# junhong-3dv/s2m2

Measured on AMD Instinct MI355X. Metric: stereo pairs/sec, S-model 1216x1024 fp16 refine_iter=3 (ms/pair = 1000*n_gpus/value), higher is better.
Workload: dtype f16; 1 GPU; S-model 1216x1024 refine_iter=3 use_positivity=True, 1 pair(s) per GPU per step, random-init weights (seeded LeCun normal); pairs_per_gpu=1, parallelism=dp1 (pairs sharded, RCCL gather of outputs to rank 0)

## Files before the change

s2m2_amd/csrc/conv.hip:

```cpp
#include "common.h"
#include "conv_select.h"
#include "launch.h"
#include "plan.h"

#ifndef S2M2_CONV_DBG
#define S2M2_CONV_DBG 0
#endif
#include "epilogue.h"

#ifndef S2M2_ASYNC_LOADS
#define S2M2_ASYNC_LOADS 0
#endif

namespace s2m2 {

struct ConvArgs {
    const void* src[4];
    int src_c[4];
    int src_stride[4];
    int nsrc;
    const void* weight;
    const float* bias;
    void* out;
    int out_stride;
    int N, H, W, KH, KW, Cin, Cout;
    int stride, Ho, Wo;
    int act, epi;
    const void* aux0;
    const void* aux1;
    int aux0_stride, aux1_stride;
    float out_scale;
    int shuffle2;
    int korder;
    const void* zero;
    const float* ln_wsum;
    float ln_eps;
    int ksplit;
    const float* bias2;
    int pool2;
    int epi_cout0;
};

template <typename T, int BM_, int BN_, int WGM_, int PPR_ = 8, int NPF_ = 1, int NWAVES_ = 4>
struct ConvCfg {
    static constexpr int NT = 64 * NWAVES_;
    static constexpr int NPF = NPF_;
    static constexpr int BM = BM_, BN = BN_, WGM = WGM_, WGN = NWAVES_ / WGM_;
    static constexpr int VEC = 16 / sizeof(T);
    static constexpr int PPR = PPR_;
    static constexpr int RPI = NT / PPR;
    static constexpr int BK = PPR * VEC;
    static constexpr int RS = BK + VEC;
    static constexpr int KSTEPS = BK / 16;
    static constexpr int WM = BM / WGM, WN = BN / WGN;
    static constexpr int MT = WM / 32, NTL = WN / 32;
    static constexpr int A_IT = (BM + RPI - 1) / RPI, B_IT = (BN + RPI - 1) / RPI;
    static constexpr int CRS = BN + VEC;
    static constexpr size_t TILE_BYTES = (size_t)2 * (BM + BN) * RS * sizeof(T);
    static constexpr size_t STAGE_BYTES = (size_t)BM * CRS * sizeof(T);
    static constexpr size_t LDS_BYTES = TILE_BYTES > STAGE_BYTES ? TILE_BYTES : STAGE_BYTES;
    static_assert(WM % 32 == 0 && WN % 32 == 0, "wave tile must be whole 32x32 MFMA tiles");
// ... 59 lines not shown
            }
            aux_combine(v, epi, a0, a1);
        }
        long long opix = m;
        int oc = co;
        if (p.shuffle2) {
            const int sub = co / p.shuffle2;
            oc = co - sub * p.shuffle2;
            const int x = (int)(m % p.Wo);
            const long long t = m / p.Wo;
            const int y = (int)(t % p.Ho);
            const long long n = t / p.Ho;
            opix = (n * (2 * p.Ho) + 2 * y + (sub >> 1)) * (2LL * p.Wo) + 2 * x + (sub & 1);
        }
        if (!(S2M2_CONV_DBG & 32)) *reinterpret_cast<Vec16<T>*>(outp + opix * p.out_stride + oc) = v;
    }
}

struct LinearPix {
    long long m0, M;
    __device__ __forceinline__ bool operator()(int r, long long& m) const { m = m0 + r; return m < M; }
};
template <int PW = 32>
struct PatchPixT {
    int n, y0, x0, H, W;
    __device__ __forceinline__ bool operator()(int r, long long& m) const {
        const int py = r / PW;
        const int yy = y0 + py, xx = x0 + (r - py * PW);
        m = ((long long)n * H + yy) * W + xx;
        return yy < H && xx < W;
    }
};
using PatchPix = PatchPixT<32>;

template <typename CFG, typename T>
__device__ __forceinline__ void stage_tile_ln(const ConvArgs& p, const float16_t (&acc)[CFG::MT][CFG::NTL], T* Cs, const CoutRegs<CFG>& bias,
                                              int wm, int wn, int lane, const LnRow* ln, const CoutRegs<CFG>& wsum) {
    if (p.act == S2M2_ACT_GELU) stage_tile<CFG, T, S2M2_ACT_GELU, true>(acc, Cs, bias, p.out_scale, wm, wn, lane, ln, &wsum);
    else stage_tile<CFG, T, S2M2_ACT_NONE, true>(acc, Cs, bias, p.out_scale, wm, wn, lane, ln, &wsum);
}

template <typename CFG, typename T>
__device__ __forceinline__ void stage_tile_act(const ConvArgs& p, const float16_t (&acc)[CFG::MT][CFG::NTL], T* Cs, const CoutRegs<CFG>& bias,
                                               int wm, int wn, int lane) {
    switch (p.act) {
        case S2M2_ACT_GELU: stage_tile<CFG, T, S2M2_ACT_GELU>(acc, Cs, bias, p.out_scale, wm, wn, lane); break;
        case S2M2_ACT_RELU: stage_tile<CFG, T, S2M2_ACT_RELU>(acc, Cs, bias, p.out_scale, wm, wn, lane); break;
        case S2M2_ACT_SIGMOID: stage_tile<CFG, T, S2M2_ACT_SIGMOID>(acc, Cs, bias, p.out_scale, wm, wn, lane); break;
        case S2M2_ACT_TANH: stage_tile<CFG, T, S2M2_ACT_TANH>(acc, Cs, bias, p.out_scale, wm, wn, lane); break;
        default: stage_tile<CFG, T, S2M2_ACT_NONE>(acc, Cs, bias, p.out_scale, wm, wn, lane); break;
    }
}

template <int CH>
struct KCursor {
    int ky, kx, kc;
    __device__ __forceinline__ void init(const ConvArgs& p, int elem) {
        ky = 0; kx = 0;
        if (p.korder) { kc = elem % CH; step(p, elem / CH); }
        else { kc = elem; norm(p); }
    }
    __device__ __forceinline__ void norm(const ConvArgs& p) {
        while (kc >= p.Cin) { kc -= p.Cin; if (++kx == p.KW) { kx = 0; ++ky; } }
    }
    __device__ __forceinline__ void step(const ConvArgs& p, int n) {
        for (int i = 0; i < n; ++i) {
            if (++kx == p.KW) { kx = 0; kc += CH; if (kc >= p.Cin) { kc -= p.Cin; ++ky; } }
        }
    }
    template <int BK> __device__ __forceinline__ void advance(const ConvArgs& p) {
        if (p.korder) step(p, BK / CH);
        else { kc += BK; norm(p); }
    }
};

template <typename CFG, typename T, bool POOL = false>
struct ConvLoader {
    static constexpr bool V1A = (S2M2_ASYNC_LOADS & 2) != 0;
    static constexpr int NQ = POOL ? 4 : 1;
    static constexpr int VEC = CFG::VEC, BK = CFG::BK, RS = CFG::RS, BN = CFG::BN;
    int pc, lrow, Ktot;
    int apix[CFG::A_IT];
    unsigned tapmask[CFG::A_IT];
    const T* wrow[CFG::B_IT];
    KCursor<4 * VEC> cur;
    const T *s0, *s1, *s2, *s3;
    int st0, st1, st2, st3, c0n, c1n, c2n;
    raw16_t ra[CFG::NPF][CFG::A_IT * NQ], rb[CFG::NPF][CFG::B_IT];

    __device__ __forceinline__ void init(const ConvArgs& p, int tid, long long m0, int n0, long long M, int Ktot_) {
        pc = tid % CFG::PPR; lrow = tid / CFG::PPR; Ktot = Ktot_;
        s0 = static_cast<const T*>(p.src[0]); s1 = static_cast<const T*>(p.src[1]);
        s2 = static_cast<const T*>(p.src[2]); s3 = static_cast<const T*>(p.src[3]);
        st0 = p.src_stride[0]; st1 = p.src_stride[1]; st2 = p.src_stride[2]; st3 = p.src_stride[3];
        c0n = p.src_c[0]; c1n = c0n + p.src_c[1]; c2n = c1n + p.src_c[2];
        const int ph = p.KH / 2, pw = p.KW / 2;
#pragma unroll
        for (int it = 0; it < CFG::A_IT; ++it) {
            const long long m = m0 + lrow + CFG::RPI * it;
            apix[it] = 0; tapmask[it] = 0u;
            if (m < M && lrow + CFG::RPI * it < CFG::BM) {
                const unsigned mu = (unsigned)m;
                const unsigned t = mu / (unsigned)p.Wo;
                const int xo = (int)(mu - t * (unsigned)p.Wo);
                const unsigned n = t / (unsigned)p.Ho;
                const int y = (int)(t - n * (unsigned)p.Ho) * p.stride, x = xo * p.stride;
// ... 748 lines not shown

#ifndef S2M2_FRAG_TRACE
#define S2M2_FRAG_TRACE 0
#endif
#if S2M2_FRAG_TRACE
__device__ unsigned long long g_frag_trace[4096 * 4 * 10];
#define FRAG_T(slot)                                                                                                          \
    do {                                                                                                                      \
        if ((threadIdx.x & 63) == 0 && blockIdx.x < 4096 && blockIdx.y == 0) {                                                \
            unsigned long long* tr_ = g_frag_trace + ((size_t)blockIdx.x * 4 + (threadIdx.x >> 6)) * 10;                     \
            tr_[(slot)] = __builtin_amdgcn_s_memtime();                                                                       \
            if ((slot) == 0) {                                                                                                \
                tr_[7] = __builtin_amdgcn_s_memrealtime();                                                                    \
                tr_[9] = (unsigned long long)__builtin_amdgcn_s_getreg((4 << 0) | (0 << 6) | (31 << 11)) |                    \
                         ((unsigned long long)__builtin_amdgcn_s_getreg((20 << 0) | (0 << 6) | (3 << 11)) << 32);             \
            }                                                                                                                 \
            if ((slot) == 6) tr_[8] = __builtin_amdgcn_s_memrealtime();                                                       \
        }                                                                                                                     \
    } while (0)
#else
#define FRAG_T(slot)
#endif

template <typename T, int BN_, int CH_, int PH_ = 4, int PW_ = 32>
struct ConvCfgF {
    static_assert(sizeof(T) == 2, "the fragment-stream kernel is fp16 only");
    static constexpr int BM = PW_ * PH_, BN = BN_, PH = PH_, PW = PW_, WGM = 1, WGN = BN_ / 32;
    static constexpr int NWAVES = WGN, NT = 64 * NWAVES;
    static constexpr int VEC = 8, CH = CH_, KS = CH_ / 16;
    static constexpr int RS = CH + VEC;
    static constexpr int WM = BM, WN = 32, MT = BM / 32, NTL = 1;
    static_assert(BM % 32 == 0, "a patch is a whole number of 32-pixel MFMA tiles");
    static constexpr int MAXHALO = (PH + 2) * (PW + 2);
    static constexpr int PPX = CH / VEC;
    static constexpr int RPI = NT / PPX;
    static constexpr int A_IT = (MAXHALO + RPI - 1) / RPI;
    static constexpr int CRS = BN + VEC;
    static constexpr int AROWS = A_IT * RPI;
    static constexpr size_t A_BYTES = (size_t)AROWS * RS * sizeof(T);
    static constexpr size_t STAGE_BYTES = (size_t)BM * CRS * sizeof(T);
    static constexpr size_t LDS_BYTES = A_BYTES > STAGE_BYTES ? A_BYTES : STAGE_BYTES;
    static_assert(NT % PPX == 0 && KS >= 2 && KS % 2 == 0, "loader geometry");
};

template <typename CFG, typename T, int AUX>
__global__ __launch_bounds__(CFG::NT) void conv_frag_kernel(ConvArgs p, int tiles_x, int tiles_y) {
    constexpr int BN = CFG::BN, VEC = CFG::VEC, RS = CFG::RS, CH = CFG::CH, KS = CFG::KS, PH = CFG::PH, PW = CFG::PW;
    extern __shared__ __attribute__((aligned(16))) char smem[];
    T* Ah = reinterpret_cast<T*>(smem);
    T* Cs = reinterpret_cast<T*>(smem);

    const int tid = threadIdx.x, lane = tid & 63;
    const int wv = __builtin_amdgcn_readfirstlane(tid >> 6);
    const int hi = lane >> 5, l31 = lane & 31;
    int bx = blockIdx.x;
    const int tx = bx % tiles_x; bx /= tiles_x;
    const int ty = bx % tiles_y;
    const int n = bx / tiles_y;
    const int y0 = ty * PH, x0 = tx * PW;
    const int n0 = blockIdx.y * BN;
    const int HW_ = p.KW + PW - 1, HH_ = p.KH + PH - 1;
    const int nhalo = HW_ * HH_;
    const int ph = p.KH / 2, pw = p.KW / 2;
    const int ntap = p.KH * p.KW;
    const int nchunk = (p.Cin + CH - 1) / CH;
    const int nfrag = nchunk * ntap * KS;
    FRAG_T(0);
    const int pc = tid % CFG::PPX, prow = tid / CFG::PPX;
    int apix[CFG::A_IT];
#pragma unroll
    for (int it = 0; it < CFG::A_IT; ++it) {
        const int hp = prow + CFG::RPI * it;
        apix[it] = -1;
        if (hp < nhalo) {
            const int hy = hp / HW_, hx = hp - hy * HW_;
            const int yy = y0 - ph + hy, xx = x0 - pw + hx;
            if (yy >= 0 && yy < p.H && xx >= 0 && xx < p.W) apix[it] = (n * p.H + yy) * p.W + xx;
        }
    }
    const T* zp = static_cast<const T*>(p.zero);
    const T* const s0 = static_cast<const T*>(p.src[0]);
    const T* const s1 = static_cast<const T*>(p.src[1]);
    const T* const s2 = static_cast<const T*>(p.src[2]);
    const T* const s3 = static_cast<const T*>(p.src[3]);
    const int st0 = p.src_stride[0], st1 = p.src_stride[1], st2 = p.src_stride[2], st3 = p.src_stride[3];
    const int c0n = p.src_c[0], c1n = c0n + p.src_c[1], c2n = c1n + p.src_c[2];
    auto load_halo = [&](int chunk) __attribute__((always_inline)) {
        const int kc = chunk * CH + pc * VEC;
        const bool cvalid = kc < p.Cin;
        const T* sp = s0;
        unsigned ss = (unsigned)st0, c = (unsigned)kc;
        if (p.nsrc > 1) {
            const bool g0 = kc >= c0n, g1 = kc >= c1n, g2 = kc >= c2n;
            const long long d1 = (const char*)s1 - (const char*)s0, d2 = (const char*)s2 - (const char*)s1, d3 = (const char*)s3 - (const char*)s2;
            sp = reinterpret_cast<const T*>((const char*)s0 + ((g0 ? d1 : 0) + (g1 ? d2 : 0) + (g2 ? d3 : 0)));
            ss = (unsigned)(st0 + (g0 ? st1 - st0 : 0) + (g1 ? st2 - st1 : 0) + (g2 ? st3 - st2 : 0));
            c = (unsigned)(kc - ((g0 ? c0n : 0) + (g1 ? c1n - c0n : 0) + (g2 ? c2n - c1n : 0)));
        }
        raw16_t ra[CFG::A_IT];
#pragma unroll
        for (int it = 0; it < CFG::A_IT; ++it) {
            const unsigned e = __umul24((unsigned)apix[it], ss) + c;
            const T* src = (cvalid && apix[it] >= 0) ? sp + e : zp;
            ra[it] = global_load16(src);
        }
#pragma unroll
        for (int it = 0; it < CFG::A_IT; ++it)
            *reinterpret_cast<raw16_t*>(Ah + (size_t)(prow + CFG::RPI * it) * RS + pc * VEC) = ra[it];
    };

    const raw16_t* wf = static_cast<const raw16_t*>(p.weight) + ((size_t)(blockIdx.y * CFG::WGN + wv) * nfrag) * 64 + lane;
    raw16_t ring[KS];

    CoutRegs<CFG> bias;
    bias.load(p.bias, p.zero, p.Cout, n0, wv, lane);
    const PatchPixT<PW> pix{n, y0, x0, p.H, p.W};
    constexpr bool AUX_LATE = AUX != 0 && PW != 32;
    using AX = AuxRegs<CFG, T, AUX != 0 ? (AUX_LATE ? 10 : 8) : 4>;
    AX aux;
    const int epi_eff = (n0 < p.epi_cout0) ? (int)S2M2_EPI_NONE : p.epi;
    if constexpr (AUX != 0 && !AUX_LATE) aux.template prefetch<AUX == 1>(p, tid, n0, pix, epi_eff);
    float16_t acc[CFG::MT][CFG::NTL];
#pragma unroll
    for (int i = 0; i < CFG::MT; ++i)
#pragma unroll
        for (int r = 0; r < 16; ++r) acc[i][0][r] = 0.f;

#pragma unroll
    for (int s = 0; s < KS; ++s) global_load16_async(ring[s], wf + (size_t)(s < nfrag ? s : nfrag - 1) * 64);
    load_halo(0);
    __syncthreads();
    FRAG_T(1);
    int g = 0;
    int poff[CFG::MT];
#pragma unroll
    for (int i = 0; i < CFG::MT; ++i) {
        if constexpr (PW == 32) poff[i] = (i * HW_ + l31) * RS;
        else { const int q = 32 * i + l31, qy = q / PW; poff[i] = (qy * HW_ + (q - qy * PW)) * RS; }
    }
    auto tap_steps = [&](int ky, int kx) __attribute__((always_inline)) {
        const T* a = Ah + (size_t)(ky * HW_ + kx) * RS + hi * 8;
        Frag<T> xf[2][CFG::MT];
#pragma unroll
        for (int i = 0; i < CFG::MT; ++i) load_frag(xf[0][i], a + poff[i]);
#pragma unroll
        for (int kk = 0; kk < KS; ++kk) {
            if (kk + 1 < KS) {
#pragma unroll
                for (int i = 0; i < CFG::MT; ++i) load_frag(xf[(kk + 1) & 1][i], a + poff[i] + (kk + 1) * 16);
            }
            wait_vmcnt<KS - 2>();
            settle(ring[kk]);
            Frag<T> wfr;
            wfr.v = __builtin_bit_cast(half8_t, ring[kk]);
#pragma unroll
            for (int i = 0; i < CFG::MT; ++i) mma32(acc[i][0], wfr, xf[kk & 1][i]);
            {
                const int f = g + KS - 1;
                global_load16_async(ring[(kk + KS - 1) % KS], wf + (size_t)(f < nfrag ? f : nfrag - 1) * 64);
            }
            ++g;
        }
    };
    for (int chunk = 0; chunk < nchunk; ++chunk) {
        if (chunk > 0) {
            wait_vmcnt<0>();
            __syncthreads();
            load_halo(chunk);
            __syncthreads();
        }
        int ky = 0, kx = 0;
#pragma unroll 1
        for (int tap = 0; tap < ntap; ++tap) {
            tap_steps(ky, kx);
            if (++kx == p.KW) { kx = 0; ++ky; }
        }
    }
    wait_vmcnt<0>();
#pragma unroll
    for (int s = 0; s < KS; ++s) settle(ring[s]);

    if constexpr (AUX_LATE) aux.template prefetch<AUX == 1>(p, tid, n0, pix, epi_eff);
    FRAG_T(2);
    __syncthreads();
    FRAG_T(3);
    stage_tile_act<CFG, T>(p, acc, Cs, bias, 0, wv, lane);
    FRAG_T(4);
    __syncthreads();
    FRAG_T(5);
    store_tile<CFG, T>(p, Cs, tid, n0, aux, pix, epi_eff);
    FRAG_T(6);
}

template <typename T, int BN_>
struct ConvCfgP {
    static constexpr int BM = 64, BN = BN_, WGM = 2, WGN = 2, NT = 256;
    static constexpr int VEC = 16 / sizeof(T);
    static constexpr int BK = 8 * VEC;
    static constexpr int RS = BK + VEC;
    static constexpr int KSTEPS = BK / 16;
    static constexpr int WM = 32, WN = BN / 2, MT = 1, NTL = WN / 32;
    static constexpr int A_IT = 2;
    static constexpr int CRS = BN + VEC;
    static constexpr size_t A_BYTES = (size_t)2 * BM * RS * sizeof(T);
    static constexpr size_t C_BYTES = (size_t)BM * CRS * sizeof(T);
    static constexpr size_t w_bytes(int K) { return (size_t)BN * (K + VEC) * sizeof(T); }
    static constexpr size_t lds_bytes(int K) { return A_BYTES + C_BYTES + w_bytes(K); }
};

template <typename CFG, typename T>
__global__ __launch_bounds__(256) void conv_pw_kernel(ConvArgs p, int ntiles) {
    constexpr int BM = CFG::BM, BN = CFG::BN, VEC = CFG::VEC, RS = CFG::RS, BK = CFG::BK;
    extern __shared__ __attribute__((aligned(16))) char smem[];
    T* As = reinterpret_cast<T*>(smem);
    T* Cs = reinterpret_cast<T*>(smem + CFG::A_BYTES);
    T* Ws = reinterpret_cast<T*>(smem + CFG::A_BYTES + CFG::C_BYTES);
    const int K = p.Cin;
    const int WRS = K + VEC;
    const int nchunk = (K + BK - 1) / BK;

    const int tid = threadIdx.x, lane = tid & 63;
    const int wv = __builtin_amdgcn_readfirstlane(tid >> 6);
    const int wm = wv & 1, wn = wv >> 1;
    const int hi = lane >> 5, l31 = lane & 31;
    const long long M = (long long)p.N * p.H * p.W;
    const int n0 = blockIdx.y * BN;
    CoutRegs<CFG> bias;
    bias.load(p.bias, p.zero, p.Cout, n0, wn, lane);
    const T* zp = static_cast<const T*>(p.zero);
// ... 324 lines not shown
```

s2m2_amd/csrc/convblock.hip:

```cpp
#include "common.h"
#include "launch.h"
#include "plan.h"
#include "epilogue.h"
#include <stdlib.h>

namespace s2m2 {

struct CbArgs {
    const half_t* x; half_t* out;
    long long xs, os;
    int N, H, W, tiles_x, tiles_y;
    const raw16_t* w1; const raw16_t* w2;
    const raw16_t* wa; const raw16_t* wb;
    const float* b1; const float* b2; const float* ba; const float* bb;
    const void* zero;
};

template <int C_, int PH_>
struct CbCfg {
    static constexpr int C = C_, PH = PH_, PW = 32, NW = C_ / 32, NT = 64 * NW, KS = 8, CH = 128, NCHUNK = C_ / 128;
    static constexpr int IH = PH + 2, IW = PW + 2, NI = IH * IW, MT1 = (NI + 31) / 32;
    static constexpr int HH = PH + 4, HW = PW + 4, NHALO = HH * HW;
    static constexpr int RS = CH + 8, TRS = C + 8;
    static constexpr int PPX = CH / 8, RPI = NT / PPX, A_IT = (NHALO + RPI - 1) / RPI, AROWS = A_IT * RPI;
    static constexpr size_t A_BYTES = (size_t)AROWS * RS * 2;
    static constexpr size_t R_BYTES = (size_t)PH * 32 * TRS * 2;
    static constexpr size_t T_BYTES = (size_t)MT1 * 32 * TRS * 2;
    static constexpr size_t A_REGION = A_BYTES > R_BYTES ? A_BYTES : R_BYTES;
    static constexpr size_t OFF_T = (A_REGION + 15) / 16 * 16, OFF_B = OFF_T + T_BYTES, LDS_BYTES = OFF_B + 4 * C * 4;
    static_assert(LDS_BYTES <= 160 * 1024 && NT % PPX == 0, "conv block tile");
};

template <int MT, int KS>
__device__ __forceinline__ void cb_steps(float16_t (&acc)[MT], const half_t* a, const int (&poff)[MT], raw16_t (&ring)[KS], const raw16_t* wf,
                                         int& g, int nfrag) {
    Frag<half_t> xf[2][MT];
#pragma unroll
    for (int i = 0; i < MT; ++i) load_frag(xf[0][i], a + poff[i]);
#pragma unroll
    for (int kk = 0; kk < KS; ++kk) {
        if (kk + 1 < KS) {
#pragma unroll
            for (int i = 0; i < MT; ++i) load_frag(xf[(kk + 1) & 1][i], a + poff[i] + (kk + 1) * 16);
        }
        wait_vmcnt<KS - 2>();
        settle(ring[kk]);
        Frag<half_t> wfr;
        wfr.v = __builtin_bit_cast(half8_t, ring[kk]);
#pragma unroll
        for (int i = 0; i < MT; ++i) mma32(acc[i], wfr, xf[kk & 1][i]);
        {
            const int f = g + KS - 1;
            global_load16_async(ring[(kk + KS - 1) % KS], wf + (size_t)(f < nfrag ? f : nfrag - 1) * 64);
        }
        ++g;
    }
}

template <typename CFG>
__global__ __launch_bounds__(CFG::NT) void conv_block_kernel(CbArgs p) {
    constexpr int C = CFG::C, PH = CFG::PH, KS = CFG::KS, RS = CFG::RS, TRS = CFG::TRS, HW = CFG::HW, IW = CFG::IW, MT1 = CFG::MT1, NCHUNK = CFG::NCHUNK;
    extern __shared__ __attribute__((aligned(16))) char smem[];
    half_t* Ah = reinterpret_cast<half_t*>(smem);
    half_t* Rt = reinterpret_cast<half_t*>(smem);
    half_t* Tt = reinterpret_cast<half_t*>(smem + CFG::OFF_T);
    float* bvec = reinterpret_cast<float*>(smem + CFG::OFF_B);
    const int tid = threadIdx.x, lane = tid & 63, l31 = lane & 31, hi = lane >> 5;
    const int wv = __builtin_amdgcn_readfirstlane(tid >> 6);
    int bx = blockIdx.x;
    const int tx = bx % p.tiles_x; bx /= p.tiles_x;
    const int ty = bx % p.tiles_y;
    const int n = bx / p.tiles_y;
    const int y0 = ty * PH, x0 = tx * 32;

    for (int i = tid; i < 4 * C; i += CFG::NT) {
        const int k = i / C, c = i - k * C;
        const float* src = k == 0 ? p.b1 : k == 1 ? p.b2 : k == 2 ? p.ba : p.bb;
        bvec[i] = src ? src[c] : 0.f;
    }
    const int pc = tid % CFG::PPX, prow = tid / CFG::PPX;
    const half_t* zp = static_cast<const half_t*>(p.zero);
    auto load_halo = [&](int chunk) __attribute__((always_inline)) {
        raw16_t ra[CFG::A_IT];
#pragma unroll
        for (int it = 0; it < CFG::A_IT; ++it) {
            const int hp = prow + CFG::RPI * it;
            const int hy = hp / HW, hx = hp - hy * HW;
            const int yy = y0 - 2 + hy, xx = x0 - 2 + hx;
            const bool ok = hp < CFG::NHALO && yy >= 0 && yy < p.H && xx >= 0 && xx < p.W;
            const half_t* src = ok ? p.x + ((long long)(n * p.H + yy) * p.W + xx) * p.xs + chunk * CFG::CH + pc * 8 : zp;
            ra[it] = global_load16(src);
        }
#pragma unroll
        for (int it = 0; it < CFG::A_IT; ++it) *reinterpret_cast<raw16_t*>(Ah + (size_t)(prow + CFG::RPI * it) * RS + pc * 8) = ra[it];
    };

    const int nfrag1 = NCHUNK * 9 * KS;
    const raw16_t* wf1 = p.w1 + (size_t)wv * nfrag1 * 64 + lane;
    const raw16_t* wfa = p.wa + (size_t)wv * (C / 16) * 64 + lane;
    raw16_t ring[KS];
    float16_t acc1[MT1], accA[PH];
#pragma unroll
    for (int i = 0; i < MT1; ++i)
#pragma unroll
        for (int r = 0; r < 16; ++r) acc1[i][r] = 0.f;
#pragma unroll
    for (int i = 0; i < PH; ++i)
#pragma unroll
        for (int r = 0; r < 16; ++r) accA[i][r] = 0.f;
    int poff1[MT1], poffA[PH];
#pragma unroll
    for (int i = 0; i < MT1; ++i) {
        int q = 32 * i + l31;
        q = q < CFG::NI ? q : CFG::NI - 1;
        const int iy = q / IW, ix = q - iy * IW;
        poff1[i] = (iy * HW + ix) * RS + hi * 8;
    }
#pragma unroll
    for (int i = 0; i < PH; ++i) poffA[i] = ((i + 2) * HW + l31 + 2) * RS + hi * 8;
#pragma unroll
    for (int s = 0; s < KS - 1; ++s) global_load16_async(ring[s], wf1 + (size_t)s * 64);
    int g = 0;
#pragma unroll 1
    for (int chunk = 0; chunk < NCHUNK; ++chunk) {
        if (chunk > 0) {
            wait_vmcnt<0>();
            __syncthreads();
        }
        load_halo(chunk);
        __syncthreads();
        int ky = 0, kx = 0;
#pragma unroll 1
        for (int tap = 0; tap < 9; ++tap) {
            cb_steps<MT1, KS>(acc1, Ah + (ky * HW + kx) * RS, poff1, ring, wf1, g, nfrag1);
            if (++kx == 3) { kx = 0; ++ky; }
        }
        wait_vmcnt<0>();
        {
            raw16_t wr[KS];
#pragma unroll
            for (int s = 0; s < KS; ++s) wr[s] = global_load16(wfa + (size_t)(chunk * KS + s) * 64);
#pragma unroll
            for (int s = 0; s < KS; ++s) {
                Frag<half_t> wfr;
                wfr.v = __builtin_bit_cast(half8_t, wr[s]);
#pragma unroll
                for (int i = 0; i < PH; ++i) {
                    Frag<half_t> xf;
                    load_frag(xf, Ah + poffA[i] + s * 16);
                    mma32(accA[i], wfr, xf);
                }
            }
        }
    }
    wait_vmcnt<0>();
#pragma unroll
    for (int s = 0; s < KS; ++s) settle(ring[s]);
    const int nfrag2 = NCHUNK * 9 * KS;
    const raw16_t* wf2 = p.w2 + (size_t)wv * nfrag2 * 64 + lane;
    __syncthreads();
#pragma unroll
    for (int i = 0; i < MT1; ++i) {
        const int q = 32 * i + l31;
        const int iy = q / IW, ix = q - iy * IW;
        const int yy = y0 - 1 + iy, xx = x0 - 1 + ix;
        const bool inside = q < CFG::NI && yy >= 0 && yy < p.H && xx >= 0 && xx < p.W;
        half_t* trow = Tt + (size_t)q * TRS + wv * 32 + 4 * hi;
#pragma unroll
        for (int gq = 0; gq < 4; ++gq) {
            const float4_t bv = *reinterpret_cast<const float4_t*>(bvec + wv * 32 + 8 * gq + 4 * hi);
            float v[4];
#pragma unroll
            for (int e = 0; e < 4; ++e) v[e] = acc1[i][4 * gq + e] + bv[e];
            const float2_t r0 = fast_gelu16x2((float2_t){v[0], v[1]}), r1 = fast_gelu16x2((float2_t){v[2], v[3]});
            half4_t h = {from_f32<half_t>(r0.x * 1.0f), from_f32<half_t>(r0.y * 1.0f), from_f32<half_t>(r1.x * 1.0f), from_f32<half_t>(r1.y * 1.0f)};
            if (!inside) h = half4_t{(half_t)0.f, (half_t)0.f, (half_t)0.f, (half_t)0.f};
            *reinterpret_cast<half4_t*>(trow + 8 * gq) = h;
        }
    }
#pragma unroll
    for (int i = 0; i < PH; ++i) {
        half_t* rrow = Rt + (size_t)(32 * i + l31) * TRS + wv * 32 + 4 * hi;
#pragma unroll
        for (int gq = 0; gq < 4; ++gq) {
            const float4_t bv = *reinterpret_cast<const float4_t*>(bvec + 2 * C + wv * 32 + 8 * gq + 4 * hi);
            half4_t h;
#pragma unroll
            for (int e = 0; e < 4; ++e) h[e] = from_f32<half_t>(fmaxf(accA[i][4 * gq + e] + bv[e], 0.f) * 1.0f);
            *reinterpret_cast<half4_t*>(rrow + 8 * gq) = h;
        }
    }
#pragma unroll
    for (int s = 0; s < KS - 1; ++s) global_load16_async(ring[s], wf2 + (size_t)s * 64);
    __syncthreads();
    float16_t acc2[PH], accB[PH];
#pragma unroll
    for (int i = 0; i < PH; ++i)
#pragma unroll
        for (int r = 0; r < 16; ++r) { acc2[i][r] = 0.f; accB[i][r] = 0.f; }
    int poff2[PH];
#pragma unroll
    for (int i = 0; i < PH; ++i) poff2[i] = (i * IW + l31) * TRS + hi * 8;
    g = 0;
#pragma unroll 1
    for (int chunk = 0; chunk < NCHUNK; ++chunk) {
        int ky = 0, kx = 0;
#pragma unroll 1
        for (int tap = 0; tap < 9; ++tap) {
            cb_steps<PH, KS>(acc2, Tt + (ky * IW + kx) * TRS + chunk * CFG::CH, poff2, ring, wf2, g, nfrag2);
            if (++kx == 3) { kx = 0; ++ky; }
        }
    }
    wait_vmcnt<0>();
#pragma unroll
    for (int s = 0; s < KS; ++s) settle(ring[s]);
    {
        const raw16_t* wfb = p.wb + (size_t)wv * (C / 16) * 64 + lane;
#pragma unroll 1
        for (int c8 = 0; c8 < C / 16; c8 += KS) {
            raw16_t wr[KS];
#pragma unroll
            for (int s = 0; s < KS; ++s) wr[s] = global_load16(wfb + (size_t)(c8 + s) * 64);
#pragma unroll
            for (int s = 0; s < KS; ++s) {
                Frag<half_t> wfr;
                wfr.v = __builtin_bit_cast(half8_t, wr[s]);
#pragma unroll
                for (int i = 0; i < PH; ++i) {
                    Frag<half_t> xf;
                    load_frag(xf, Rt + (size_t)(32 * i + l31) * TRS + hi * 8 + (c8 + s) * 16);
                    mma32(accB[i], wfr, xf);
                }
            }
        }
    }
#pragma unroll
    for (int i = 0; i < PH; ++i) {
        const int yy = y0 + i, xx = x0 + l31;
        if (yy < p.H && xx < p.W) {
            half_t* orow = p.out + ((long long)(n * p.H + yy) * p.W + xx) * p.os + wv * 32 + 4 * hi;
#pragma unroll
            for (int gq = 0; gq < 4; ++gq) {
                const float4_t b2 = *reinterpret_cast<const float4_t*>(bvec + C + wv * 32 + 8 * gq + 4 * hi);
                const float4_t bb = *reinterpret_cast<const float4_t*>(bvec + 3 * C + wv * 32 + 8 * gq + 4 * hi);
                half4_t h;
#pragma unroll
                for (int e = 0; e < 4; ++e) {
                    const half_t m = from_f32<half_t>((acc2[i][4 * gq + e] + b2[e]) * 1.0f);
                    const half_t s1 = from_f32<half_t>((accB[i][4 * gq + e] + bb[e]) * 1.0f);
                    h[e] = from_f32<half_t>((float)m + (float)s1);
                }
                *reinterpret_cast<half4_t*>(orow + 8 * gq) = h;
            }
        }
    }
}

template <int C, int PH>
static int launch_cb(const CbArgs& a0, hipStream_t st) {
    using CFG = CbCfg<C, PH>;
    CbArgs a = a0;
    a.tiles_x = (a.W + 31) / 32;
    a.tiles_y = (a.H + PH - 1) / PH;
    return launch<conv_block_kernel<CFG>>("conv_block", dim3((unsigned)(a.N * a.tiles_x * a.tiles_y)), dim3(CFG::NT), CFG::LDS_BYTES, st, a);
}

}

extern "C" int s2m2_conv_block_supported(int C, int H, int W, int dtype) {
    return dtype == S2M2_F16 && (C == 128 || C == 256) && H >= 1 && W >= 1 && (long long)H * W <= 160 * 192;
}

static int conv_block_impl(const s2m2_convblock_desc* d, void* stream) {
    using namespace s2m2;
    S2M2_REQUIRE(d, "conv_block: null descriptor");
    S2M2_REQUIRE(d->dtype == S2M2_F16 && (d->C == 128 || d->C == 256), "conv_block: C=%d dtype=%d (fp16, C = 128 / 256)", d->C, d->dtype);
    S2M2_REQUIRE(d->x && d->out && d->x != d->out, "conv_block: x / out must be distinct non-null tensors");
    S2M2_REQUIRE(d->N > 0 && d->H > 0 && d->W > 0 && (long long)d->N * d->H * d->W < (1LL << 24), "conv_block: bad shape");
    S2M2_REQUIRE(d->x_stride >= d->C && d->x_stride % 8 == 0 && d->out_stride >= d->C && d->out_stride % 4 == 0, "conv_block: pixel strides");
    S2M2_REQUIRE(d->w_conv0 && d->w_conv2 && d->w_1x0 && d->w_1x2, "conv_block: null weight");
    CbArgs a;
    a.x = static_cast<const half_t*>(d->x); a.out = static_cast<half_t*>(d->out); a.xs = d->x_stride; a.os = d->out_stride;
    a.N = d->N; a.H = d->H; a.W = d->W;
    a.w1 = static_cast<const raw16_t*>(d->w_conv0); a.w2 = static_cast<const raw16_t*>(d->w_conv2);
    a.wa = static_cast<const raw16_t*>(d->w_1x0); a.wb = static_cast<const raw16_t*>(d->w_1x2);
    a.b1 = d->b_conv0; a.b2 = d->b_conv2; a.ba = d->b_1x0; a.bb = d->b_1x2;
    if (bind_zero_page(a, "conv_block")) return 1;
    hipStream_t st = static_cast<hipStream_t>(stream);
    if (d->C == 256) return launch_cb<256, 2>(a, st);
    const long long b4 = (long long)d->N * ((d->W + 31) / 32) * ((d->H + 3) / 4);
    return (d->patch_rows == 4 || (d->patch_rows != 2 && b4 >= 128)) ? launch_cb<128, 4>(a, st) : launch_cb<128, 2>(a, st);
}
extern "C" int s2m2_conv_block(const s2m2_convblock_desc* d, void* stream) {
    return s2m2::plan_dispatch_desc<s2m2_convblock_desc>("s2m2_conv_block", &conv_block_impl, d, stream);
}

S2M2_PLAN_DESC_ENTRY("s2m2_conv_block", conv_block_impl)
```

Measured before the change: 125.4 pairs/s.

## Switch fragment-streaming conv kernels to 16x16x32 MFMA with paired weight steps

```diff
diff --git a/s2m2_amd/csrc/conv.hip b/s2m2_amd/csrc/conv.hip
--- a/s2m2_amd/csrc/conv.hip
+++ b/s2m2_amd/csrc/conv.hip
@@ -7,6 +7,8 @@
 #define S2M2_CONV_DBG 0
 #endif
 #include "epilogue.h"
+#include "frag_stream.h"
+#include <type_traits>
 
 #ifndef S2M2_ASYNC_LOADS
 #define S2M2_ASYNC_LOADS 0
@@ -172,6 +174,17 @@
     }
 }
 
+template <typename CFG, typename T, int NTILE>
+__device__ __forceinline__ void stage_tile_act(const ConvArgs& p, const float4_t (&acc)[NTILE][2], T* Cs, const CoutRegs16& bias, int, int wn, int lane) {
+    switch (p.act) {
+        case S2M2_ACT_GELU: stage_tile16<CFG, T, S2M2_ACT_GELU>(acc, Cs, bias, p.out_scale, wn, lane); break;
+        case S2M2_ACT_RELU: stage_tile16<CFG, T, S2M2_ACT_RELU>(acc, Cs, bias, p.out_scale, wn, lane); break;
+        case S2M2_ACT_SIGMOID: stage_tile16<CFG, T, S2M2_ACT_SIGMOID>(acc, Cs, bias, p.out_scale, wn, lane); break;
+        case S2M2_ACT_TANH: stage_tile16<CFG, T, S2M2_ACT_TANH>(acc, Cs, bias, p.out_scale, wn, lane); break;
+        default: stage_tile16<CFG, T, S2M2_ACT_NONE>(acc, Cs, bias, p.out_scale, wn, lane); break;
+    }
+}
+
 template <int CH>
 struct KCursor {
     int ky, kx, kc;
@@ -1026,7 +1039,6 @@
 
     const int tid = threadIdx.x, lane = tid & 63;
     const int wv = __builtin_amdgcn_readfirstlane(tid >> 6);
-    const int hi = lane >> 5, l31 = lane & 31;
     int bx = blockIdx.x;
     const int tx = bx % tiles_x; bx /= tiles_x;
     const int ty = bx % tiles_y;
@@ -1086,7 +1098,9 @@
     const raw16_t* wf = static_cast<const raw16_t*>(p.weight) + ((size_t)(blockIdx.y * CFG::WGN + wv) * nfrag) * 64 + lane;
     raw16_t ring[KS];
 
-    CoutRegs<CFG> bias;
+    using FS = FragShape<FRAG_MFMA>;
+    constexpr int NTILE = CFG::BM / FS::PIX;
+    std::conditional_t<FRAG_MFMA == 16, CoutRegs16, CoutRegs<CFG>> bias;
     bias.load(p.bias, p.zero, p.Cout, n0, wv, lane);
     const PatchPixT<PW> pix{n, y0, x0, p.H, p.W};
     constexpr bool AUX_LATE = AUX != 0 && PW != 32;
@@ -1094,61 +1108,47 @@
     AX aux;
     const int epi_eff = (n0 < p.epi_cout0) ? (int)S2M2_EPI_NONE : p.epi;
     if constexpr (AUX != 0 && !AUX_LATE) aux.template prefetch<AUX == 1>(p, tid, n0, pix, epi_eff);
-    float16_t acc[CFG::MT][CFG::NTL];
-#pragma unroll
-    for (int i = 0; i < CFG::MT; ++i)
-#pragma unroll
-        for (int r = 0; r < 16; ++r) acc[i][0][r] = 0.f;
-
-#pragma unroll
-    for (int s = 0; s < KS; ++s) global_load16_async(ring[s], wf + (size_t)(s < nfrag ? s : nfrag - 1) * 64);
-    load_halo(0);
-    __syncthreads();
-    FRAG_T(1);
+    typename FS::acc_t acc[NTILE];
+#pragma unroll
+    for (int i = 0; i < NTILE; ++i) frag_zero<FRAG_MFMA>(acc[i]);
+
+    if constexpr (FRAG_MFMA == 32) {
+#pragma unroll
+        for (int s = 0; s < KS; ++s) global_load16_async(ring[s], wf + (size_t)(s < nfrag ? s : nfrag - 1) * 64);
+        load_halo(0);
+        __syncthreads();
+        FRAG_T(1);
+    }
     int g = 0;
-    int poff[CFG::MT];
-#pragma unroll
-    for (int i = 0; i < CFG::MT; ++i) {
-        if constexpr (PW == 32) poff[i] = (i * HW_ + l31) * RS;
-        else { const int q = 32 * i + l31, qy = q / PW; poff[i] = (qy * HW_ + (q - qy * PW)) * RS; }
-    }
-    auto tap_steps = [&](int ky, int kx) __attribute__((always_inline)) {
-        const T* a = Ah + (size_t)(ky * HW_ + kx) * RS + hi * 8;
-        Frag<T> xf[2][CFG::MT];
-#pragma unroll
-        for (int i = 0; i < CFG::MT; ++i) load_frag(xf[0][i], a + poff[i]);
-#pragma unroll
-        for (int kk = 0; kk < KS; ++kk) {
-            if (kk + 1 < KS) {
-#pragma unroll
-                for (int i = 0; i < CFG::MT; ++i) load_frag(xf[(kk + 1) & 1][i], a + poff[i] + (kk + 1) * 16);
-            }
-            wait_vmcnt<KS - 2>();
-            settle(ring[kk]);
-            Frag<T> wfr;
-            wfr.v = __builtin_bit_cast(half8_t, ring[kk]);
-#pragma unroll
-            for (int i = 0; i < CFG::MT; ++i) mma32(acc[i][0], wfr, xf[kk & 1][i]);
-            {
-                const int f = g + KS - 1;
-                global_load16_async(ring[(kk + KS - 1) % KS], wf + (size_t)(f < nfrag ? f : nfrag - 1) * 64);
-            }
-            ++g;
-        }
-    };
+    int poff[NTILE];
+    const int lpx = FS::pixel(lane), lko = FS::koff(lane);
+#pragma unroll
+    for (int i = 0; i < NTILE; ++i) {
+        const int q = FS::PIX * i + lpx, qy = q / PW;
+        poff[i] = (qy * HW_ + (q - qy * PW)) * RS + lko;
+    }
     for (int chunk = 0; chunk < nchunk; ++chunk) {
-        if (chunk > 0) {
-            wait_vmcnt<0>();
-            __syncthreads();
+        if constexpr (FRAG_MFMA == 32) {
+            if (chunk > 0) {
+                wait_vmcnt<0>();
+                __syncthreads();
+                load_halo(chunk);
+                __syncthreads();
+            }
+        } else {
+            if (chunk > 0) __syncthreads();
+            frag_prime<FRAG_MFMA, KS>(ring, wf, g, nfrag);
             load_halo(chunk);
             __syncthreads();
+            if (chunk == 0) FRAG_T(1);
         }
         int ky = 0, kx = 0;
 #pragma unroll 1
-        for (int tap = 0; tap < ntap; ++tap) {
-            tap_steps(ky, kx);
+        for (int tap = 0; tap < (FRAG_MFMA == 32 ? ntap : ntap - 1); ++tap) {
+            frag_steps<FRAG_MFMA, NTILE, KS>(acc, Ah + (size_t)(ky * HW_ + kx) * RS, poff, ring, wf, g, nfrag);
             if (++kx == p.KW) { kx = 0; ++ky; }
         }
+        if constexpr (FRAG_MFMA == 16) frag_steps<FRAG_MFMA, NTILE, KS, FRAG_MFMA == 16>(acc, Ah + (size_t)(ky * HW_ + kx) * RS, poff, ring, wf, g, nfrag);
     }
     wait_vmcnt<0>();
 #pragma unroll
diff --git a/s2m2_amd/csrc/convblock.hip b/s2m2_amd/csrc/convblock.hip
--- a/s2m2_amd/csrc/convblock.hip
+++ b/s2m2_amd/csrc/convblock.hip
@@ -2,6 +2,7 @@
 #include "launch.h"
 #include "plan.h"
 #include "epilogue.h"
+#include "frag_stream.h"
 #include <stdlib.h>
 
 namespace s2m2 {
@@ -26,46 +27,26 @@
     static constexpr size_t A_BYTES = (size_t)AROWS * RS * 2;
     static constexpr size_t R_BYTES = (size_t)PH * 32 * TRS * 2;
     static constexpr size_t T_BYTES = (size_t)MT1 * 32 * TRS * 2;
+    using FS = FragShape<FRAG_MFMA>;
+    static constexpr int NT1 = (NI + FS::PIX - 1) / FS::PIX;
+    static constexpr int NT2 = PH * 32 / FS::PIX;
+    static_assert(NT1 * FS::PIX <= MT1 * 32, "the intermediate's rows");
     static constexpr size_t A_REGION = A_BYTES > R_BYTES ? A_BYTES : R_BYTES;
     static constexpr size_t OFF_T = (A_REGION + 15) / 16 * 16, OFF_B = OFF_T + T_BYTES, LDS_BYTES = OFF_B + 4 * C * 4;
     static_assert(LDS_BYTES <= 160 * 1024 && NT % PPX == 0, "conv block tile");
 };
 
-template <int MT, int KS>
-__device__ __forceinline__ void cb_steps(float16_t (&acc)[MT], const half_t* a, const int (&poff)[MT], raw16_t (&ring)[KS], const raw16_t* wf,
-                                         int& g, int nfrag) {
-    Frag<half_t> xf[2][MT];
-#pragma unroll
-    for (int i = 0; i < MT; ++i) load_frag(xf[0][i], a + poff[i]);
-#pragma unroll
-    for (int kk = 0; kk < KS; ++kk) {
-        if (kk + 1 < KS) {
-#pragma unroll
-            for (int i = 0; i < MT; ++i) load_frag(xf[(kk + 1) & 1][i], a + poff[i] + (kk + 1) * 16);
-        }
-        wait_vmcnt<KS - 2>();
-        settle(ring[kk]);
-        Frag<half_t> wfr;
-        wfr.v = __builtin_bit_cast(half8_t, ring[kk]);
-#pragma unroll
-        for (int i = 0; i < MT; ++i) mma32(acc[i], wfr, xf[kk & 1][i]);
-        {
-            const int f = g + KS - 1;
-            global_load16_async(ring[(kk + KS - 1) % KS], wf + (size_t)(f < nfrag ? f : nfrag - 1) * 64);
-        }
-        ++g;
-    }
-}
-
 template <typename CFG>
 __global__ __launch_bounds__(CFG::NT) void conv_block_kernel(CbArgs p) {
-    constexpr int C = CFG::C, PH = CFG::PH, KS = CFG::KS, RS = CFG::RS, TRS = CFG::TRS, HW = CFG::HW, IW = CFG::IW, MT1 = CFG::MT1, NCHUNK = CFG::NCHUNK;
+    constexpr int C = CFG::C, PH = CFG::PH, KS = CFG::KS, RS = CFG::RS, TRS = CFG::TRS, HW = CFG::HW, IW = CFG::IW, NT1 = CFG::NT1, NT2 = CFG::NT2, NCHUNK = CFG::NCHUNK;
+    using FS = typename CFG::FS;
     extern __shared__ __attribute__((aligned(16))) char smem[];
     half_t* Ah = reinterpret_cast<half_t*>(smem);
     half_t* Rt = reinterpret_cast<half_t*>(smem);
     half_t* Tt = reinterpret_cast<half_t*>(smem + CFG::OFF_T);
     float* bvec = reinterpret_cast<float*>(smem + CFG::OFF_B);
     const int tid = threadIdx.x, lane = tid & 63, l31 = lane & 31, hi = lane >> 5;
+    const int lpx = FS::pixel(lane), lko = FS::koff(lane), lq = lane >> 4;
     const int wv = __builtin_amdgcn_readfirstlane(tid >> 6);
     int bx = blockIdx.x;
     const int tx = bx % p.tiles_x; bx /= p.tiles_x;
@@ -99,42 +80,42 @@
     const raw16_t* wf1 = p.w1 + (size_t)wv * nfrag1 * 64 + lane;
     const raw16_t* wfa = p.wa + (size_t)wv * (C / 16) * 64 + lane;
     raw16_t ring[KS];
-    float16_t acc1[MT1], accA[PH];
-#pragma unroll
-    for (int i = 0; i < MT1; ++i)
-#pragma unroll
-        for (int r = 0; r < 16; ++r) acc1[i][r] = 0.f;
+    typename FS::acc_t acc1[NT1];
+    float16_t accA[PH];
+#pragma unroll
+    for (int i = 0; i < NT1; ++i) frag_zero<FRAG_MFMA>(acc1[i]);
 #pragma unroll
     for (int i = 0; i < PH; ++i)
 #pragma unroll
         for (int r = 0; r < 16; ++r) accA[i][r] = 0.f;
-    int poff1[MT1], poffA[PH];
-#pragma unroll
-    for (int i = 0; i < MT1; ++i) {
-        int q = 32 * i + l31;
+    int poff1[NT1], poffA[PH];
+#pragma unroll
+    for (int i = 0; i < NT1; ++i) {
+        int q = FS::PIX * i + lpx;
         q = q < CFG::NI ? q : CFG::NI - 1;
         const int iy = q / IW, ix = q - iy * IW;
-        poff1[i] = (iy * HW + ix) * RS + hi * 8;
+        poff1[i] = (iy * HW + ix) * RS + lko;
     }
 #pragma unroll
     for (int i = 0; i < PH; ++i) poffA[i] = ((i + 2) * HW + l31 + 2) * RS + hi * 8;
-#pragma unroll
-    for (int s = 0; s < KS - 1; ++s) global_load16_async(ring[s], wf1 + (size_t)s * 64);
     int g = 0;
+    if constexpr (FRAG_MFMA == 32) frag_prime<FRAG_MFMA, KS>(ring, wf1, 0, nfrag1);
 #pragma unroll 1
     for (int chunk = 0; chunk < NCHUNK; ++chunk) {
         if (chunk > 0) {
             wait_vmcnt<0>();
             __syncthreads();
         }
+        if constexpr (FRAG_MFMA == 16) frag_prime<FRAG_MFMA, KS>(ring, wf1, g, nfrag1);
         load_halo(chunk);
         __syncthreads();
         int ky = 0, kx = 0;
 #pragma unroll 1
-        for (int tap = 0; tap < 9; ++tap) {
-            cb_steps<MT1, KS>(acc1, Ah + (ky * HW + kx) * RS, poff1, ring, wf1, g, nfrag1);
+        for (int tap = 0; tap < (FRAG_MFMA == 32 ? 9 : 8); ++tap) {
+            frag_steps<FRAG_MFMA, NT1, KS>(acc1, Ah + (ky * HW + kx) * RS, poff1, ring, wf1, g, nfrag1);
             if (++kx == 3) { kx = 0; ++ky; }
         }
+        if constexpr (FRAG_MFMA == 16) frag_steps<FRAG_MFMA, NT1, KS, FRAG_MFMA == 16>(acc1, Ah + (2 * HW + 2) * RS, poff1, ring, wf1, g, nfrag1);
         wait_vmcnt<0>();
         {
             raw16_t wr[KS];
@@ -160,22 +141,27 @@
     const raw16_t* wf2 = p.w2 + (size_t)wv * nfrag2 * 64 + lane;
     __syncthreads();
 #pragma unroll
-    for (int i = 0; i < MT1; ++i) {
-        const int q = 32 * i + l31;
+    for (int i = 0; i < NT1; ++i) {
+        const int q = FS::PIX * i + lpx;
         const int iy = q / IW, ix = q - iy * IW;
         const int yy = y0 - 1 + iy, xx = x0 - 1 + ix;
         const bool inside = q < CFG::NI && yy >= 0 && yy < p.H && xx >= 0 && xx < p.W;
-        half_t* trow = Tt + (size_t)q * TRS + wv * 32 + 4 * hi;
-#pragma unroll
-        for (int gq = 0; gq < 4; ++gq) {
-            const float4_t bv = *reinterpret_cast<const float4_t*>(bvec + wv * 32 + 8 * gq + 4 * hi);
+        constexpr int NQ = FRAG_MFMA == 32 ? 4 : 2, QS = 32 / NQ;
+        const int c0 = wv * 32 + 4 * (FRAG_MFMA == 32 ? hi : lq);
+        half_t* trow = Tt + (size_t)q * TRS + c0;
+#pragma unroll
+        for (int gq = 0; gq < NQ; ++gq) {
+            const float4_t bv = *reinterpret_cast<const float4_t*>(bvec + c0 + QS * gq);
             float v[4];
 #pragma unroll
-            for (int e = 0; e < 4; ++e) v[e] = acc1[i][4 * gq + e] + bv[e];
+            for (int e = 0; e < 4; ++e) {
+                if constexpr (FRAG_MFMA == 32) v[e] = acc1[i][0][4 * gq + e] + bv[e];
+                else v[e] = acc1[i][gq][e] + bv[e];
+            }
             const float2_t r0 = fast_gelu16x2((float2_t){v[0], v[1]}), r1 = fast_gelu16x2((float2_t){v[2], v[3]});
             half4_t h = {from_f32<half_t>(r0.x * 1.0f), from_f32<half_t>(r0.y * 1.0f), from_f32<half_t>(r1.x * 1.0f), from_f32<half_t>(r1.y * 1.0f)};
             if (!inside) h = half4_t{(half_t)0.f, (half_t)0.f, (half_t)0.f, (half_t)0.f};
-            *reinterpret_cast<half4_t*>(trow + 8 * gq) = h;
+            *reinterpret_cast<half4_t*>(trow + QS * gq) = h;
         }
     }
 #pragma unroll
@@ -191,25 +177,31 @@
         }
     }
 #pragma unroll
-    for (int s = 0; s < KS - 1; ++s) global_load16_async(ring[s], wf2 + (size_t)s * 64);
+    for (int s = 0; s < FS::primed(KS); ++s) global_load16_async(ring[s], wf2 + (size_t)s * 64);
     __syncthreads();
-    float16_t acc2[PH], accB[PH];
+    typename FS::acc_t acc2[NT2];
+    float16_t accB[PH];
+#pragma unroll
+    for (int i = 0; i < NT2; ++i) frag_zero<FRAG_MFMA>(acc2[i]);
 #pragma unroll
     for (int i = 0; i < PH; ++i)
 #pragma unroll
-        for (int r = 0; r < 16; ++r) { acc2[i][r] = 0.f; accB[i][r] = 0.f; }
-    int poff2[PH];
-#pragma unroll
-    for (int i = 0; i < PH; ++i) poff2[i] = (i * IW + l31) * TRS + hi * 8;
+        for (int r = 0; r < 16; ++r) accB[i][r] = 0.f;
+    int poff2[NT2];
+#pragma unroll
+    for (int i = 0; i < NT2; ++i) {
+        const int q = FS::PIX * i + lpx;
+        poff2[i] = ((q >> 5) * IW + (q & 31)) * TRS + lko;
+    }
     g = 0;
+    {
+        int ky = 0, kx = 0, coff = 0;
 #pragma unroll 1
-    for (int chunk = 0; chunk < NCHUNK; ++chunk) {
-        int ky = 0, kx = 0;
-#pragma unroll 1
-        for (int tap = 0; tap < 9; ++tap) {
-            cb_steps<PH, KS>(acc2, Tt + (ky * IW + kx) * TRS + chunk * CFG::CH, poff2, ring, wf2, g, nfrag2);
-            if (++kx == 3) { kx = 0; ++ky; }
-        }
+        for (int tap = 0; tap < NCHUNK * 9 - (FRAG_MFMA == 32 ? 0 : 1); ++tap) {
+            frag_steps<FRAG_MFMA, NT2, KS>(acc2, Tt + (ky * IW + kx) * TRS + coff, poff2, ring, wf2, g, nfrag2);
+            if (++kx == 3) { kx = 0; if (++ky == 3) { ky = 0; coff += CFG::CH; } }
+        }
+        if constexpr (FRAG_MFMA == 16) frag_steps<FRAG_MFMA, NT2, KS, FRAG_MFMA == 16>(acc2, Tt + (2 * IW + 2) * TRS + (NCHUNK - 1) * CFG::CH, poff2, ring, wf2, g, nfrag2);
     }
     wait_vmcnt<0>();
 #pragma unroll
@@ -234,6 +226,24 @@
             }
         }
     }
+    if constexpr (FRAG_MFMA == 16) {
+        __syncthreads();
+#pragma unroll
+        for (int i = 0; i < NT2; ++i) {
+            half_t* mrow = Tt + (size_t)(16 * i + lpx) * TRS + wv * 32 + 4 * lq;
+#pragma unroll
+            for (int gq = 0; gq < 2; ++gq) {
+                const float4_t b2 = *reinterpret_cast<const float4_t*>(bvec + C + wv * 32 + 16 * gq + 4 * lq);
+                half4_t h;
+#pragma unroll
+                for (int e = 0; e < 4; ++e) h[e] = from_f32<half_t>((acc2[i][gq][e] + b2[e]) * 1.0f);
+                *reinterpret_cast<half4_t*>(mrow + 16 * gq) = h;
+            }
+        }
+        __builtin_amdgcn_fence(__ATOMIC_RELEASE, "wavefront");
+        __builtin_amdgcn_wave_barrier();
+        __builtin_amdgcn_fence(__ATOMIC_ACQUIRE, "wavefront");
+    }
 #pragma unroll
     for (int i = 0; i < PH; ++i) {
         const int yy = y0 + i, xx = x0 + l31;
@@ -243,10 +253,13 @@
             for (int gq = 0; gq < 4; ++gq) {
                 const float4_t b2 = *reinterpret_cast<const float4_t*>(bvec + C + wv * 32 + 8 * gq + 4 * hi);
                 const float4_t bb = *reinterpret_cast<const float4_t*>(bvec + 3 * C + wv * 32 + 8 * gq + 4 * hi);
-                half4_t h;
+                half4_t h, m4;
+                if constexpr (FRAG_MFMA == 16) m4 = *reinterpret_cast<const half4_t*>(Tt + (size_t)(32 * i + l31) * TRS + wv * 32 + 4 * hi + 8 * gq);
 #pragma unroll
                 for (int e = 0; e < 4; ++e) {
-                    const half_t m = from_f32<half_t>((acc2[i][4 * gq + e] + b2[e]) * 1.0f);
+                    half_t m;
+                    if constexpr (FRAG_MFMA == 16) m = m4[e];
+                    else m = from_f32<half_t>((acc2[i][0][4 * gq + e] + b2[e]) * 1.0f);
                     const half_t s1 = from_f32<half_t>((accB[i][4 * gq + e] + bb[e]) * 1.0f);
                     h[e] = from_f32<half_t>((float)m + (float)s1);
                 }
diff --git a/s2m2_amd/csrc/frag_stream.h b/s2m2_amd/csrc/frag_stream.h
--- /dev/null
+++ b/s2m2_amd/csrc/frag_stream.h
@@ -0,0 +1,169 @@
+#pragma once
+#include "common.h"
+#include "epilogue.h"
+
+#ifndef S2M2_FRAG_MFMA
+#define S2M2_FRAG_MFMA 16
+#endif
+static_assert(S2M2_FRAG_MFMA == 16 || S2M2_FRAG_MFMA == 32, "S2M2_FRAG_MFMA: 16 (v_mfma_f32_16x16x32_f16) or 32 (v_mfma_f32_32x32x16_f16)");
+
+namespace s2m2 {
+
+constexpr int FRAG_MFMA = S2M2_FRAG_MFMA;
+
+template <int SHAPE> struct FragShape;
+template <> struct FragShape<32> {
+    static constexpr int PIX = 32;
+    typedef float16_t acc_t[1];
+    __device__ static __forceinline__ int pixel(int lane) { return lane & 31; }
+    __device__ static __forceinline__ int koff(int lane) { return (lane >> 5) * 8; }
+    static constexpr int primed(int ks) { return ks - 1; }
+};
+template <> struct FragShape<16> {
+    static constexpr int PIX = 16;
+    typedef float4_t acc_t[2];
+    __device__ static __forceinline__ int pixel(int lane) {
+        const int c = lane & 15;
+        return (c >= 4 && c < 12) ? 2 * (c - 4) : (c < 4 ? 2 * c + 1 : 2 * (c - 8) + 1);
+    }
+    __device__ static __forceinline__ int koff(int lane) { const int q = lane >> 4; return (q & 1) * 16 + (q >> 1) * 8; }
+    static constexpr int primed(int ks) { return ks - 2; }
+};
+
+template <int SHAPE> __device__ __forceinline__ void frag_zero(typename FragShape<SHAPE>::acc_t& a) {
+    if constexpr (SHAPE == 32) {
+#pragma unroll
+        for (int r = 0; r < 16; ++r) a[0][r] = 0.f;
+    } else {
+#pragma unroll
+        for (int r = 0; r < 4; ++r) { a[0][r] = 0.f; a[1][r] = 0.f; }
+    }
+}
+
+template <int SHAPE, int KS>
+__device__ __forceinline__ void frag_prime(raw16_t (&ring)[KS], const raw16_t* wf, int g, int nfrag) {
+#pragma unroll
+    for (int s = 0; s < FragShape<SHAPE>::primed(KS); ++s) global_load16_async(ring[s], wf + (size_t)(g + s < nfrag ? g + s : nfrag - 1) * 64);
+}
+
+__device__ __forceinline__ void frag_pair_swap(raw16_t& f0, raw16_t& f1) {
+#pragma unroll
+    for (int d = 0; d < 4; ++d) {
+        const float a0 = f0[d], a1 = f1[d];
+        const auto r = __builtin_amdgcn_permlane16_swap(__builtin_bit_cast(unsigned, a0), __builtin_bit_cast(unsigned, a1), false, false);
+        const unsigned u0 = r[0], u1 = r[1];
+        f0[d] = __builtin_bit_cast(float, u0);
+        f1[d] = __builtin_bit_cast(float, u1);
+    }
+}
+
+template <int SHAPE, int NTILE, int KS, bool LAST = false>
+__device__ __forceinline__ void frag_steps(typename FragShape<SHAPE>::acc_t (&acc)[NTILE], const half_t* a, const int (&poff)[NTILE], raw16_t (&ring)[KS],
+                                           const raw16_t* wf, int& g, int nfrag) {
+    if constexpr (SHAPE == 32) {
+        static_assert(!LAST, "the 32-wide loop keeps its ring in flight across taps and chunks");
+        Frag<half_t> xf[2][NTILE];
+#pragma unroll
+        for (int i = 0; i < NTILE; ++i) load_frag(xf[0][i], a + poff[i]);
+#pragma unroll
+        for (int kk = 0; kk < KS; ++kk) {
+            if (kk + 1 < KS) {
+#pragma unroll
+                for (int i = 0; i < NTILE; ++i) load_frag(xf[(kk + 1) & 1][i], a + poff[i] + (kk + 1) * 16);
+            }
+            wait_vmcnt<KS - 2>();
+            settle(ring[kk]);
+            Frag<half_t> wfr;
+            wfr.v = __builtin_bit_cast(half8_t, ring[kk]);
+#pragma unroll
+            for (int i = 0; i < NTILE; ++i) mma32(acc[i][0], wfr, xf[kk & 1][i]);
+            {
+                const int f = g + KS - 1;
+                global_load16_async(ring[(kk + KS - 1) % KS], wf + (size_t)(f < nfrag ? f : nfrag - 1) * 64);
+            }
+            ++g;
+        }
+    } else {
+        static_assert(KS % 2 == 0 && KS >= 4, "k16 steps are consumed in pairs (half-empty chunks read zeros: the pairs are always complete)");
+        constexpr int H0 = (NTILE + 1) / 2;
+        Frag<half_t> xf[2][H0];
+#pragma unroll
+        for (int i = 0; i < H0; ++i) load_frag(xf[0][i], a + poff[i]);
+#pragma unroll
+        for (int kk = 0; kk < KS; kk += 2) {
+#pragma unroll
+            for (int i = H0; i < NTILE; ++i) load_frag(xf[1][i - H0], a + poff[i] + kk * 16);
+            wait_vmcnt_n((LAST && KS - 2 - kk < KS - 4) ? KS - 2 - kk : KS - 4);
+            settle(ring[kk]);
+            settle(ring[kk + 1]);
+            frag_pair_swap(ring[kk], ring[kk + 1]);
+            Frag<half_t> w0, w1;
+            w0.v = __builtin_bit_cast(half8_t, ring[kk]);
+            w1.v = __builtin_bit_cast(half8_t, ring[kk + 1]);
+#pragma unroll
+            for (int i = 0; i < H0; ++i) {
+                acc[i][0] = __builtin_amdgcn_mfma_f32_16x16x32_f16(w0.v, xf[0][i].v, acc[i][0], 0, 0, 0);
+                acc[i][1] = __builtin_amdgcn_mfma_f32_16x16x32_f16(w1.v, xf[0][i].v, acc[i][1], 0, 0, 0);
+            }
+            if (!LAST || kk == 0) {
+#pragma unroll
+                for (int s = 0; s < 2; ++s) {
+                    const int f = g + KS - 2 + s;
+                    global_load16_async(ring[(kk + KS - 2 + s) % KS], wf + (size_t)(f < nfrag ? f : nfrag - 1) * 64);
+                }
+            }
+            if (kk + 2 < KS) {
+#pragma unroll
+                for (int i = 0; i < H0; ++i) load_frag(xf[0][i], a + poff[i] + (kk + 2) * 16);
+            }
+#pragma unroll
+            for (int i = H0; i < NTILE; ++i) {
+                acc[i][0] = __builtin_amdgcn_mfma_f32_16x16x32_f16(w0.v, xf[1][i - H0].v, acc[i][0], 0, 0, 0);
+                acc[i][1] = __builtin_amdgcn_mfma_f32_16x16x32_f16(w1.v, xf[1][i - H0].v, acc[i][1], 0, 0, 0);
+            }
+            g += 2;
+        }
+    }
+}
+
+struct CoutRegs16 {
+    raw16_t v[2];
+    __device__ __forceinline__ void load(const float* src, const void* zero, int Cout, int n0, int wn, int lane) {
+#pragma unroll
+        for (int h = 0; h < 2; ++h) {
+            const int co = n0 + wn * 32 + 16 * h + 4 * (lane >> 4);
+            const float* q = (src != nullptr && co < Cout) ? src + co : static_cast<const float*>(zero);
+            v[h] = global_load16(q);
+        }
+    }
+};
+
+template <typename CFG, typename T, int ACT, int NTILE>
+__device__ __forceinline__ void stage_tile16(const float4_t (&acc)[NTILE][2], T* Cs, const CoutRegs16& bias, float out_scale, int wn, int lane) {
+    static_assert(sizeof(T) == 2, "the fragment-stream family is fp16");
+    const int px = FragShape<16>::pixel(lane);
+#pragma unroll
+    for (int t = 0; t < NTILE; ++t) {
+        T* crow = Cs + (size_t)(16 * t + px) * CFG::CRS + wn * 32 + 4 * (lane >> 4);
+#pragma unroll
+        for (int h = 0; h < 2; ++h) {
+            const raw16_t bv = bias.v[h];
+            float v[4];
+#pragma unroll
+            for (int e = 0; e < 4; ++e) v[e] = acc[t][h][e] + bv[e];
+            if constexpr (ACT == S2M2_ACT_GELU && S2M2_GELU16_POLY) {
+                if (!(S2M2_CONV_DBG & 16)) {
+                    const float2_t r0 = fast_gelu16x2((float2_t){v[0], v[1]}), r1 = fast_gelu16x2((float2_t){v[2], v[3]});
+                    v[0] = r0.x * out_scale; v[1] = r0.y * out_scale; v[2] = r1.x * out_scale; v[3] = r1.y * out_scale;
+                }
+            } else {
+#pragma unroll
+                for (int e = 0; e < 4; ++e) v[e] = (S2M2_CONV_DBG & 16) ? acc[t][h][e] : activate<ACT>(v[e]) * out_scale;
+            }
+            half4_t hv = {from_f32<half_t>(v[0]), from_f32<half_t>(v[1]), from_f32<half_t>(v[2]), from_f32<half_t>(v[3])};
+            *reinterpret_cast<half4_t*>(crow + 16 * h) = hv;
+        }
+    }
+}
+
+}
```

Result: no change. 126.7 pairs/s (median of 6 runs) (+1.0%).
